# julius-speech/julius

Hardware: NVIDIA H100
Metric: frames/sec (xRT) 20k-word triphone decode (higher is better)
Workload: dtype f32

## Files before the change

### julius_b200/csrc/beam.cu

```cuda
#include "common.cuh"
#include "heap_pipe.cuh"
#include <vector>
#include <algorithm>

struct jb200_gmm;
struct jb200_dnn;
namespace jb200 {
int dnn_forward_device(jb200_dnn *h, const float *d_in, int T, float *d_rows, int row_stride, cudaStream_t st);
int gmm_device(const jb200_gmm *h);
int gmm_dim(const jb200_gmm *h);
int gmm_launch_states(jb200_gmm *h, const float *d_feats, int T, float *d_rows, int row_stride, cudaStream_t st,
                      const int *seg_off, const int *seg_start, int n_seg);
int gmm_cd_device(const jb200_gmm *h, const int **cd_off, const int **cd_states, int *method, int *nbest);

static constexpr int BEAM_THREADS = 256;
static constexpr int NWARP = BEAM_THREADS / 32;
static constexpr int SEQ_LOCAL_BITS = 18;
static constexpr unsigned SEQ_LOCAL = 1u << SEQ_LOCAL_BITS;
static constexpr int CD_NMAX = 16;
static constexpr int MAX_WORDS = 150;

struct __align__(16) NodeRec { float self_a, next_a; int arc_off, arc_n; int stend, next; int scid, out; };
struct __align__(8) Tok { float score; int node; int tre; int cword; float lscore; int tre_wid; };
struct __align__(16) Cand { float score; int node; float lscore; int src; };
// ... 162 lines not shown
        }
      }
      if (n < maxn) n++;
    }
  }
  float prob = 0.0f;
  for (int i = 0; i < n; i++) prob += mp[i];
  return prob / (float)n;
}

__device__ __forceinline__ float outprob_style(const BeamParams &p, const float *__restrict__ row, int out, int last_wid) {
  const int style = (unsigned)out >> 28, ref = out & 0x0fffffff;
  if (style == JB200_AS_STATE) return __ldg(row + ref);
  if (style == JB200_AS_LSET) return cdset_score(p, row, ref);
  const int col = (last_wid < 0) ? p.n_ctx : __ldg(p.word_ctx + last_wid);
  const int r = __ldg(p.rset_ctx + (size_t)ref * (p.n_ctx + 1) + col);
  if (r >= 0) return __ldg(row + r);
  return cdset_score(p, row, -r - 1);
}

__device__ __forceinline__ int block_excl_scan(int v, int *warp_sums, int *total) {
  const int lane = threadIdx.x & 31, wid = threadIdx.x >> 5;
  int x = v;
#pragma unroll
  for (int o = 1; o < 32; o <<= 1) { int y = __shfl_up_sync(0xffffffffu, x, o); if (lane >= o) x += y; }
  if (lane == 31) warp_sums[wid] = x;
  __syncthreads();
  if (wid == 0) {
    int s = (lane < NWARP) ? warp_sums[lane] : 0;
#pragma unroll
    for (int o = 1; o < 32; o <<= 1) { int y = __shfl_up_sync(0xffffffffu, s, o); if (lane >= o) s += y; }
    if (lane < NWARP) warp_sums[lane] = s;
  }
  __syncthreads();
  const int base = (wid == 0) ? 0 : warp_sums[wid - 1];
  *total = warp_sums[NWARP - 1];
  const int r = base + x - v;
  __syncthreads();
  return r;
}

__device__ __forceinline__ void cand_atomics(const SlotView &slots,
                                             int node, float score, unsigned seq_first, unsigned seq_win) {
  atomicMin(slots.fs(node), (int)seq_first);
  unsigned long long key = ((unsigned long long)fkey(score) << 32) | (unsigned)(~seq_win);
  atomicMax(slots.bk(node), key);
}

__device__ __forceinline__ float hval(unsigned long long e) { return __uint_as_float((unsigned)(e & 0xffffffffu)); }

template <bool MAXHEAP>
__device__ __forceinline__ bool hcmp(float a, float b) { return MAXHEAP ? (a < b) : (a > b); }
template <bool MAXHEAP>
__device__ __forceinline__ bool hstop(float s, float c) { return MAXHEAP ? (s >= c) : (s <= c); }

template <bool MAXHEAP>
__device__ __forceinline__ void sift_down(unsigned long long *A, int start, int n) {
  const unsigned long long s = A[start];
  const float sv = hval(s);
  int parent = start, child;
  while ((child = parent * 2) <= n) {
    const ulonglong2 pr = *reinterpret_cast<const ulonglong2 *>(A + child);
    unsigned long long c = pr.x;
    if (child < n && hcmp<MAXHEAP>(hval(pr.x), hval(pr.y))) { child++; c = pr.y; }
    if (hstop<MAXHEAP>(sv, hval(c))) break;
    A[parent] = c;
    parent = child;
  }
  A[parent] = s;
}

template <bool MAXHEAP>
__device__ __forceinline__ void sift_root_2level(unsigned long long *A, const unsigned long long s, const int m) {
  const float sv = hval(s);
  int parent = 1;
  while (true) {
    int child = parent * 2;
    if (child > m) break;
    const ulonglong2 pr = *reinterpret_cast<const ulonglong2 *>(A + child);
    const int g = parent * 4;
    ulonglong2 g01 = make_ulonglong2(0ull, 0ull), g23 = make_ulonglong2(0ull, 0ull);
    if (g <= m) g01 = *reinterpret_cast<const ulonglong2 *>(A + g);
    if (g + 2 <= m) g23 = *reinterpret_cast<const ulonglong2 *>(A + g + 2);
    unsigned long long c = pr.x; bool right = false;
    if (child < m && hcmp<MAXHEAP>(hval(pr.x), hval(pr.y))) { right = true; c = pr.y; }
    if (hstop<MAXHEAP>(sv, hval(c))) break;
    A[parent] = c;
    parent = child + (right ? 1 : 0);
    child = parent * 2;
    if (child > m) break;
    const ulonglong2 q = right ? g23 : g01;
    unsigned long long c2 = q.x; bool right2 = false;
    if (child < m && hcmp<MAXHEAP>(hval(q.x), hval(q.y))) { right2 = true; c2 = q.y; }
    if (hstop<MAXHEAP>(sv, hval(c2))) break;
    A[parent] = c2;
    parent = child + (right2 ? 1 : 0);
  }
  A[parent] = s;
}

template <bool MAXHEAP>
__device__ void heap_build(unsigned long long *A, int n) {
  const int half = n >> 1;
  if (half >= 1) {
    for (int L = 31 - __clz(half); L >= 0; L--) {
      const int lo = 1 << L;
      const int hi = min((2 << L) - 1, half);
      for (int i = lo + (int)threadIdx.x; i <= hi; i += BEAM_THREADS) sift_down<MAXHEAP>(A, i, n);
      __syncthreads();
    }
  }
}

template <bool MAXHEAP>
__device__ void heap_extract_seq(unsigned long long *A, int n, int extract) {
  if (threadIdx.x == 0) {
    int m = n;
    while (m > n - extract) {
      const unsigned long long s = A[m];
      A[m] = A[1];
      m--;
      if (m >= 1) sift_root_2level<MAXHEAP>(A, s, m);
    }
  }
  __syncthreads();
}

__device__ __forceinline__ ulonglong2 ldcg_pair(const unsigned long long *p) {
  const uint4 v = __ldcg(reinterpret_cast<const uint4 *>(p));
  return make_ulonglong2(((unsigned long long)v.y << 32) | v.x, ((unsigned long long)v.w << 32) | v.z);
}
struct HeapCache {
  unsigned long long *top; int cs;
  unsigned long long *tail; int tail_first, tail_n;
};

template <bool MAXHEAP>
__device__ void heap_extract_pipe_global(unsigned long long *A, const int n, const int extract, const float lose_below,
                                         unsigned long long *outs, const int maxt, const HeapCache hc,
                                         unsigned &ticks_out, unsigned &stalls_out) {
  constexpr int NL = 16;
  constexpr unsigned FULL = 0xffffffffu;
  const unsigned lane = threadIdx.x & 31;
  const unsigned long long sent = MAXHEAP ? 0xff800000ull : 0x7f800000ull;
  const int cap = (maxt >> 1) + 1;
  auto load_slot = [&](int i) -> unsigned long long {
    if (i < hc.cs) return hc.top[i];
    if (i >= hc.tail_first && i < hc.tail_first + hc.tail_n) return hc.tail[i - hc.tail_first];
    return __ldcg(A + i);
  };
  auto store_slot = [&](int i, unsigned long long v) {
    __stcg(A + i, v);
    if (i < hc.cs) hc.top[i] = v;
    else if (i >= hc.tail_first && i < hc.tail_first + hc.tail_n) hc.tail[i - hc.tail_first] = v;
  };
  bool act = false;
  int slot = 0, cur = cap, my_x = 0;
  unsigned long long s = sent;
  int next_x = 0, wait = 0;
  unsigned ticks = 0, stalls = 0;
  if (lane == 0 && extract > 0) outs[0] = load_slot(1);
  unsigned long long nxt = load_slot(n);
  while (true) {
    ulonglong2 pr = make_ulonglong2(sent, sent);
    if (act) {
      const int i = 2 * cur;
      if (i + 1 < hc.cs) pr = *reinterpret_cast<const ulonglong2 *>(hc.top + i);
      else if (i >= hc.tail_first && i + 1 < hc.tail_first + hc.tail_n) pr = make_ulonglong2(hc.tail[i - hc.tail_first], hc.tail[i + 1 - hc.tail_first]);
      else pr = ldcg_pair(A + i);
    }
    if (act) {
      const float xv = hval(pr.x), yv = hval(pr.y), sv = hval(s);
      const bool right = hcmp<MAXHEAP>(xv, yv);
      const unsigned long long c = right ? pr.y : pr.x;
      const float cv = hval(c);
      const bool stop = hstop<MAXHEAP>(sv, cv) || (MAXHEAP && cv < lose_below);
      const unsigned long long put = stop ? s : c;
      store_slot(slot, put);
      if (slot == 1) outs[my_x + 1] = put;
      if (stop) act = false;
      else { slot = 2 * cur + (right ? 1 : 0); cur = min(slot, cap); }
    }
    __syncwarp();
    if (--wait <= 0) {
      if (next_x >= extract) { if (!__any_sync(FULL, act)) break; }
      else {
        const int ms = n - next_x;
        const int ln = next_x & (NL - 1);
        bool blocks = act && ((int)lane == ln);
        if (!(MAXHEAP && hval(nxt) < lose_below)) {
          const int dh = 31 - __clz(max(slot, 1)), dms = 31 - __clz(ms);
          blocks = blocks || (act && dms >= dh && (ms >> (dms - dh)) == slot);
        }
        if (!__any_sync(FULL, blocks)) {
          if ((int)lane == ln) {
            s = load_slot(ms);
            store_slot(ms, sent);
            my_x = next_x; act = true; slot = 1; cur = 1;
          }
          next_x++; wait = 2;
          nxt = load_slot(n - next_x);
        } else stalls++;
      }
    }
    __syncwarp();
    ticks++;
  }
  ticks_out = ticks; stalls_out = stalls;
}

struct SlotClear {
  const Tok *tok; int n; SlotView slots;
  __device__ __forceinline__ void run(int first, int stride) const {
    for (int i = first; i < n; i += stride) {
      const int node = tok[i].node;
      slots.reset(node);
    }
  }
};

template <bool MAXHEAP>
__device__ __forceinline__ void heap_pad_sentinels(unsigned long long *A, const int n, const int maxt) {
  const unsigned long long sent = MAXHEAP ? 0xff800000ull : 0x7f800000ull;
  const int hi = min(2 * n + 1, maxt + 1);
  for (int i = n + 1 + (int)threadIdx.x; i <= hi; i += BEAM_THREADS) A[i] = sent;
  if (threadIdx.x < 2) A[maxt + 2 + threadIdx.x] = sent;
}

extern __shared__ __align__(16) unsigned char beam_smem[];
struct CutAreas {
  unsigned long long *heap;
  int *offs;
  unsigned long long *gq; int gqn;
  unsigned long long *gtail; int gtn;
  __device__ __forceinline__ unsigned long long *outv() const { return reinterpret_cast<unsigned long long *>(offs); }
};
__device__ __forceinline__ CutAreas cut_areas(const BeamParams &p) {
  unsigned long long *const smem_q = reinterpret_cast<unsigned long long *>(beam_smem);
  CutAreas a;
  a.heap = p.heap_g ? p.heap_g + (size_t)blockIdx.x * (p.maxt + 4) : smem_q;
  a.offs = reinterpret_cast<int *>(smem_q + (p.heap_g ? p.qcap : p.maxt + 4));
  a.gq = p.heap_g ? smem_q : nullptr;
  a.gqn = p.heap_g ? p.qcap : 0;
  a.gtail = p.heap_g ? reinterpret_cast<unsigned long long *>(a.offs + 2 * (p.beam + 2)) : nullptr;
  a.gtn = p.heap_g ? p.beam + 1 : 0;
  return a;
}

template <bool MAXHEAP>
__device__ void heap_extract_fast(const CutAreas &ca, const int n, const int extract, const float lose_below, const int maxt,
                                  unsigned long long *stats, const SlotClear *idle_work = nullptr) {
  unsigned long long *const A = ca.heap, *const outv = ca.outv(), *const gcache = ca.gq;
  HeapCache hc{nullptr, 0, nullptr, 0, 0};
  if (!__isShared(A) && n + 8 <= ca.gqn) {
    const int lmaxt = (ca.gqn - 4) & ~1;
    for (int i = threadIdx.x; i <= n; i += BEAM_THREADS) gcache[i] = A[i];
    heap_pad_sentinels<MAXHEAP>(gcache, n, lmaxt);
    __syncthreads();
    if (threadIdx.x >= 32 && idle_work) idle_work->run((int)threadIdx.x - 32, BEAM_THREADS - 32);
    if (threadIdx.x < 32) {
      unsigned ticks, stalls;
      heap_extract_pipe_warp6<MAXHEAP>(gcache, n, extract, lose_below, outv, lmaxt, threadIdx.x, ticks, stalls);
      if (threadIdx.x == 0) {
        atomicAdd(stats + CUT_REPLAY_TICKS, (unsigned long long)ticks); atomicAdd(stats + CUT_REPLAY_EXTRACTS, (unsigned long long)extract);
        atomicAdd(stats + CUT_HELD_BACK, (unsigned long long)stalls); atomicAdd(stats + CUT_GLOBAL_WHOLE, 1ull);
      }
    }
    __syncthreads();
    for (int i = 1 + threadIdx.x; i <= n; i += BEAM_THREADS) A[i] = gcache[i];
    __syncthreads();
    return;
  }
  if (!__isShared(A)) {
    hc.top = gcache; hc.cs = min(ca.gqn, maxt + 4) & ~1;
    for (int i = threadIdx.x; i < hc.cs; i += BEAM_THREADS) gcache[i] = A[i];
    if (ca.gtn >= extract) {
      hc.tail = ca.gtail; hc.tail_first = n - extract + 1; hc.tail_n = extract;
      for (int i = threadIdx.x; i < extract; i += BEAM_THREADS) ca.gtail[i] = A[hc.tail_first + i];
    }
    __syncthreads();
  }
  if (threadIdx.x >= 32 && idle_work) idle_work->run((int)threadIdx.x - 32, BEAM_THREADS - 32);
  if (threadIdx.x < 32) {
    unsigned ticks, stalls;
    if (!__isShared(A)) heap_extract_pipe_global<MAXHEAP>(A, n, extract, lose_below, outv, maxt, hc, ticks, stalls);
    else heap_extract_pipe_warp6<MAXHEAP>(A, n, extract, lose_below, outv, maxt, threadIdx.x, ticks, stalls);
    if (threadIdx.x == 0) {
      atomicAdd(stats + CUT_REPLAY_TICKS, (unsigned long long)ticks); atomicAdd(stats + CUT_REPLAY_EXTRACTS, (unsigned long long)extract);
      atomicAdd(stats + CUT_HELD_BACK, (unsigned long long)stalls);
      if (!__isShared(A)) atomicAdd(stats + CUT_GLOBAL_TOP_TAIL, 1ull);
    }
  }
  __syncthreads();
}

__device__ __forceinline__ int closed_subtree_size(const int c, const int n, const int H) {
  const int dc = 31 - __clz(c);
  if (dc > H) return 0;
  const int sh = H - dc;
  const int first = c << sh, width = 1 << sh;
  return (width - 1) + max(0, min(n - first + 1, width));
}

__device__ __noinline__ int closed_relocate(unsigned long long *keys, const int nc, const int n, const int need, unsigned *flags, unsigned *multi,
                                            unsigned *pay, const int lane) {
  constexpr unsigned FULL = 0xffffffffu;
  const int H = 31 - __clz(n);
  const int tail0 = n - need + 1, fwords = (need + 31) >> 5;
  for (int w = fwords - 1; w >= 0; w--) {
    unsigned bits = flags[w];
    while (bits) {
      const int b = 31 - __clz(bits);
      const int m = tail0 + w * 32 + b;
      const int k = n - m + 1;
      if (m <= n && m >= 2 && k <= need) {
        const int dm = 31 - __clz(m);
        const bool is_multi = (multi[(m - tail0) >> 5] >> ((m - tail0) & 31)) & 1u;
        int j = 0, a = 1, lo = 0, hi = n, occ = -1;
        bool gone = false;
        for (int base = k - 1; base < nc && occ < 0 && !gone; base += 32) {
          const int idx = base + lane;
          const unsigned long long key = (idx < nc) ? keys[idx] : 0ull;
          const int pre = 0xffff - (int)((key >> 16) & 0xffffu);
          unsigned done = 0u;
          while (true) {
            const bool in = (idx < nc) && pre >= lo && pre < hi && !((done >> lane) & 1u);
            const unsigned mask = __ballot_sync(FULL, in);
            if (!mask) break;
            const int f = __ffs(mask) - 1;
            if (j == dm) { occ = base + f; break; }
            if (!is_multi && (int)(pay[(unsigned)keys[base + f] & 0xffffu] >> 16) == m) { gone = true; break; }
            j++;
            const int nxt = m >> (dm - j);
            const int lsz = closed_subtree_size(2 * a, n, H);
            if (nxt == 2 * a) { lo = lo + 1; hi = lo + lsz; } else { lo = lo + 1 + lsz; }
            a = nxt;
            done |= (f >= 31) ? FULL : ((2u << f) - 1u);
          }
        }
        if (occ >= k) {
          __syncwarp();
          const unsigned long long ekey = keys[occ];
          const unsigned esc = (unsigned)(ekey >> 32);
          const int msz = m - 1;
          int x = 1; lo = 0; hi = n;
          bool stop = (2 * x > msz);
          for (int base = k; base < nc && !stop; base += 32) {
            const int idx = base + lane;
            const unsigned long long key = (idx < nc) ? keys[idx] : 0ull;
            const int pre = 0xffff - (int)((key >> 16) & 0xffffu);
            unsigned done = 0u;
            while (!stop) {
              const bool in = (idx < nc) && idx != occ && pre >= lo && pre < hi && !((done >> lane) & 1u);
              const unsigned mask = __ballot_sync(FULL, in);
              if (!mask) break;
              const int f = __ffs(mask) - 1;
              const unsigned osc = __shfl_sync(FULL, (unsigned)(key >> 32), f);
              const int opre = __shfl_sync(FULL, pre, f);
              if (opre == lo) return 0;
              if (esc >= osc) { stop = true; break; }
              const int lsz = closed_subtree_size(2 * x, n, H);
              if (opre < lo + 1 + lsz) { x = 2 * x; lo = lo + 1; hi = lo + lsz; }
              else { x = 2 * x + 1; lo = lo + 1 + lsz; }
              if (2 * x > msz) { stop = true; break; }
              done |= (f >= 31) ? FULL : ((2u << f) - 1u);
            }
          }
          const unsigned long long nkey = (ekey & 0xffffffff0000ffffull) | ((unsigned long long)(0xffffu - (unsigned)lo) << 16);
          int cnt = 0;
          {
            const int wb = max(k, occ - 16), we = wb + 31;
            const bool lo_ok = (wb == k) || ((unsigned)(keys[wb] >> 32) > esc);
            const bool hi_ok = (we >= nc) || ((unsigned)(keys[we] >> 32) < esc);
            if (lo_ok && hi_ok) {
              const int idx = wb + lane;
              const bool gt = (idx < nc) && idx != occ && keys[idx] > nkey;
              cnt = (wb - k) + __popc(__ballot_sync(FULL, gt));
            } else {
              for (int base = k; base < nc; base += 32) {
                const int idx = base + lane;
                const bool gt = (idx < nc) && idx != occ && keys[idx] > nkey;
                const unsigned mask = __ballot_sync(FULL, gt);
                cnt += __popc(mask);
                const bool le = (idx < nc) && idx != occ && !gt;
                if (__any_sync(FULL, le)) break;
              }
            }
          }
          const int ins = k + cnt;
          if (ins < occ) {
            for (int top = occ; top > ins; top -= 32) {
              const int idx = top - lane;
              unsigned long long v = 0ull;
              if (idx > ins) v = keys[idx - 1];
              __syncwarp();
              if (idx > ins) keys[idx] = v;
              __syncwarp();
            }
          } else if (ins > occ) {
            for (int bot = occ; bot < ins; bot += 32) {
              const int idx = bot + lane;
              unsigned long long v = 0ull;
              if (idx < ins) v = keys[idx + 1];
              __syncwarp();
              if (idx < ins) keys[idx] = v;
              __syncwarp();
            }
          }
          if (lane == 0) {
            keys[ins] = nkey;
            unsigned *pp = pay + ((unsigned)nkey & 0xffffu);
            *pp = ((unsigned)x << 16) | (*pp & 0xffffu);
            if (x >= tail0 && x < m) { flags[(x - tail0) >> 5] |= 1u << ((x - tail0) & 31); multi[(x - tail0) >> 5] |= 1u << ((x - tail0) & 31); }
          }
          __syncwarp();
        }
      }
      bits = flags[w] & ((b == 0) ? 0u : ((1u << b) - 1u));
    }
  }
  return 1;
}

__device__ int heap_select_closed(unsigned long long *heap, const int n, const int need, const float lose_below, const int maxt,
                                  unsigned long long *keys, const int key_cap, unsigned *pay, const int pay_cap,
                                  int *ordn, int *s_scratch ) {
  const int tid = threadIdx.x;
  int relocated = 0;
  if (n >= 65536 || maxt >= 65536 || !(lose_below > -INFINITY)) return 0;
  const int tail0 = n - need + 1, fwords = (need + 31) >> 5;
  unsigned *const flags = pay + pay_cap - fwords, *const multi = pay + pay_cap - 2 * fwords;
  const bool have_flags = (2 * fwords < pay_cap);
  if (tid == 0) { s_scratch[0] = 0; s_scratch[1] = 0; }
  if (have_flags) for (int i = tid; i < 2 * fwords; i += BEAM_THREADS) multi[i] = 0u;
  __syncthreads();
  const int H = 31 - __clz(n);
  const int cap = min(min(key_cap, have_flags ? pay_cap - 2 * fwords : pay_cap), 65535);
  for (int h0 = 1; h0 <= n; h0 += BEAM_THREADS) {
    const int h = h0 + tid;
    unsigned long long e = 0ull;
    bool is_c = false;
    if (h <= n) { e = heap[h]; is_c = (hval(e) >= lose_below); }
    const unsigned m = __ballot_sync(0xffffffffu, is_c);
    int base = 0;
    if ((tid & 31) == 0 && m) base = atomicAdd(&s_scratch[0], __popc(m));
    base = __shfl_sync(0xffffffffu, base, 0);
    if (is_c) {
      const int ci = base + __popc(m & ((1u << (tid & 31)) - 1u));
      if (ci < cap) {
        int pre = 0, cur = 1;
        for (int b = (31 - __clz(h)) - 1; b >= 0; b--) {
          const int bit = (h >> b) & 1;
          pre += 1 + (bit ? closed_subtree_size(cur * 2, n, H) : 0);
          cur = cur * 2 + bit;
        }
        keys[ci] = ((unsigned long long)fkey(hval(e)) << 32) | ((unsigned long long)(0xffffu - (unsigned)pre) << 16) | (unsigned)ci;
        pay[ci] = ((unsigned)h << 16) | (unsigned)(e >> 32);
      }
    }
  }
  __syncthreads();
  const int nc = s_scratch[0];
  int np = 1; while (np < nc) np <<= 1;
  if (nc > cap || np > key_cap || nc < need) return 0;
  const bool can_relocate = have_flags;
  for (int i = nc + tid; i < np; i += BEAM_THREADS) keys[i] = 0ull;
  __syncthreads();
  for (int k = 2; k <= np; k <<= 1) {
    for (int j = k >> 1; j > 0; j >>= 1) {
      for (int i = tid; i < (np >> 1); i += BEAM_THREADS) {
        const int a = ((i & ~(j - 1)) << 1) | (i & (j - 1)), b = a | j;
        const unsigned long long ka = keys[a], kb = keys[b];
        const bool desc = ((a & k) == 0);
        if (desc ? (ka < kb) : (ka > kb)) { keys[a] = kb; keys[b] = ka; }
      }
      __syncthreads();
    }
  }
  const unsigned theta = (unsigned)(keys[need - 1] >> 32);
  for (int i = tid; i < nc; i += BEAM_THREADS) {
    const unsigned long long ki = keys[i];
    const unsigned sk = (unsigned)(ki >> 32);
    if (sk < theta) continue;
    const int slot = (int)(pay[(unsigned)ki & 0xffffu] >> 16);
    if (slot < tail0) continue;
    const bool tied = (i > 0 && (unsigned)(keys[i - 1] >> 32) == sk) || (i + 1 < nc && (unsigned)(keys[i + 1] >> 32) == sk);
    int last = i;
    if (tied) { int g = 0; while (last + 1 < nc && (unsigned)(keys[last + 1] >> 32) == sk && g < 8) { last++; g++; } if (g == 8) last = nc; }
    const int kstep = n - slot + 1, d = 31 - __clz(slot);
    if (last + 1 < kstep + d) continue;
    if (have_flags) atomicOr(flags + ((slot - tail0) >> 5), 1u << ((slot - tail0) & 31));
    if (tied) s_scratch[1] = 1;
  }
  __syncthreads();
  if (s_scratch[1]) {
    if (!can_relocate) return 0;
    if (tid < 32) { const int ok = closed_relocate(keys, nc, n, need, flags, multi, pay, tid); if (tid == 0) s_scratch[1] = ok ? 2 : 1; }
    __syncthreads();
    if (s_scratch[1] != 2) return 0;
    relocated = 1;
  }
  for (int k = tid; k < need; k += BEAM_THREADS) ordn[k] = (int)(pay[(unsigned)keys[need - 1 - k] & 0xffffu] & 0xffffu);
  return 1 + relocated;
}


__device__ int trace_backptr(const jb200_atom *atoms, int a, int *w) {
  int n = 0;
  w[n++] = atoms[a].wid;
  while (atoms[a].begintime > 0) {
    a = atoms[a].last;
    if (a < 0 || n >= MAX_WORDS) break;
    w[n++] = atoms[a].wid;
  }
  for (int i = 0; i < n / 2; i++) { const int x = w[i]; w[i] = w[n - 1 - i]; w[n - 1 - i] = x; }
  return n;
}

__device__ void interim_best(const BeamParams &p, const int u, const jb200_atom *araw, const int lo, const int hi, const int frame) {
  UttState *st = p.state + u;
  int best = -1; float mx = JB200_LOG_ZERO;
  for (int a = hi - 1; a >= lo; a--) if (mx < araw[a].backscore) { mx = araw[a].backscore; best = a; }
  st->interim_frame = frame - 1;
  if (best < 0) { st->interim_nwords = 0; st->interim_score = JB200_LOG_ZERO; return; }
  st->interim_nwords = trace_backptr(araw, best, p.interim_words + (size_t)u * MAX_WORDS); st->interim_score = mx;
}

#define PROF_MARK(k) do { if (tid == 0) { long long _n = clock64(); s_prof[k] += _n - s_tprev; s_tprev = _n; } } while (0)

__device__ __forceinline__ void beam_cut(const BeamParams &p, const CutAreas &ca, const int n, const unsigned &s_maxkey,
                                         const Tok *tn, const SlotView &slots, int *ordn, long long *s_prof, long long &s_tprev) {
  __shared__ unsigned s_losekey;
  __shared__ int s_cf[2];
  const int tid = threadIdx.x;
  const int need = p.beam, maxt = p.maxt;
  unsigned long long *const heap = ca.heap, *const outv = ca.outv();
  const SlotClear sc{tn, n, slots};
  if (need < n - need) {
    constexpr int NB = 1024;
    int *hist = ca.offs;
    const int nb = min(NB, 2 * (p.beam + 2));
    for (int i = tid; i < nb; i += BEAM_THREADS) hist[i] = 0;
    __syncthreads();
    const unsigned maxkey = s_maxkey;
    const int e = (int)((((maxkey & 0x80000000u) ? (maxkey & 0x7fffffffu) : ~maxkey) >> 23) & 0xffu) - 127;
    const int sh = max(0, min(24, 22 - e));
    for (int r = tid; r < n; r += BEAM_THREADS) {
      const unsigned key = fkey(hval(heap[r + 1]));
      const unsigned bin = min((unsigned)(nb - 1), (maxkey - key) >> sh);
      atomicAdd(&hist[bin], 1);
    }
    __syncthreads();
    if (tid < 32) {
      int cum = 0, found = -1;
      for (int b0 = 0; b0 < nb && found < 0; b0 += 32) {
        const int v = (b0 + tid < nb) ? hist[b0 + tid] : 0;
        int x = v;
        for (int o = 1; o < 32; o <<= 1) { int y = __shfl_up_sync(0xffffffffu, x, o); if (tid >= o) x += y; }
        const unsigned hit = __ballot_sync(0xffffffffu, cum + x >= need);
        if (hit) found = b0 + __ffs(hit) - 1;
        cum += __shfl_sync(0xffffffffu, x, 31);
      }
      if (tid == 0) {
        unsigned lk = 0u;
        if (found >= 0 && found < nb - 1) {
          const unsigned long long drop = (unsigned long long)(found + 1) << sh;
          lk = (drop < maxkey) ? maxkey - (unsigned)drop : 0u;
        }
        s_losekey = lk;
      }
    }
    __syncthreads();
    const unsigned lk = s_losekey;
    const float lose_below = (lk == 0u) ? -INFINITY : __uint_as_float((lk & 0x80000000u) ? (lk & 0x7fffffffu) : ~lk);
    heap_build<true>(heap, n); PROF_MARK(7);
    sc.run(tid, BEAM_THREADS);
    const int closed = heap_select_closed(heap, n, need, lose_below, maxt, ca.gq ? ca.gq : heap + n + 1, ca.gq ? p.sort_cap : maxt + 3 - n,
                                          reinterpret_cast<unsigned *>(ca.offs), 2 * (p.beam + 2), ordn, s_cf);
    if (tid == 0) {
      atomicAdd(p.cut_counters + CUT_UPWARD, 1ull);
      if (closed) atomicAdd(p.cut_counters + CUT_CLOSED, 1ull);
      if (closed == 2) atomicAdd(p.cut_counters + CUT_RELOCATED, 1ull);
    }
    if (!closed) {
      heap_pad_sentinels<true>(heap, n, maxt);
      __syncthreads();
      heap_extract_fast<true>(ca, n, need, lose_below, maxt, p.cut_counters);
      for (int k = tid; k < need; k += BEAM_THREADS) ordn[k] = (int)(outv[need - 1 - k] >> 32);
    }
  } else {
    heap_pad_sentinels<false>(heap, n, maxt);
    heap_build<false>(heap, n); PROF_MARK(7);
    heap_extract_fast<false>(ca, n, n - need, -INFINITY, maxt, p.cut_counters, &sc);
    for (int k = tid; k < need; k += BEAM_THREADS) ordn[k] = (int)(heap[k + 1] >> 32);
  }
}

template <bool GRAMMAR>
__device__ __forceinline__ void finalize_utt(const BeamParams &p, const int u, const int tid, const int T, jb200_atom *araw, int *newidx,
                                             const int *group0, jb200_utt_result *res, int *words,
                                             int &s_natoms, int &s_overflow, int &s_found, long long &s_outbase,
                                             long long *s_prof, long long &s_tprev) {
  const int natoms = s_natoms;
  for (int a = tid; a < natoms; a += BEAM_THREADS) {
    const jb200_atom me = araw[a];
    const int lo = group0[me.endtime], hi = group0[me.endtime + 1];
    int rank = 0;
    for (int b = lo; b < hi; b++) rank += (araw[b].wid < me.wid) ? 1 : 0;
    newidx[a] = lo + rank;
  }
  if (tid == 0) {
    if (p.atoms_in_place) s_outbase = p.atom_off[u];
    else {
      unsigned long long base = atomicAdd(p.atom_counter, (unsigned long long)natoms);
      if ((long long)(base + natoms) > p.atoms_out_cap) { s_overflow = 1; s_outbase = -1; }
      else s_outbase = (long long)base;
    }
  }
  __syncthreads();
  const long long ob = s_outbase;
  const bool can_write = (ob >= 0);
  const int kept = can_write ? natoms : 0;
  for (int a = tid; a < kept; a += BEAM_THREADS) {
    jb200_atom me = araw[a];
    me.last = (me.last < 0) ? -1 : newidx[me.last];
    p.atoms_out[ob + newidx[a]] = me;
    if ((GRAMMAR || me.wid == p.tail_silwid) && me.backscore > JB200_LOG_ZERO) atomicMax(&s_found, me.endtime);
  }
  __threadfence_block();
  __syncthreads();

  if (tid == 0) {
    int status = 0, nw = 0; float score = 0.0f;
    const int last_time = s_found;
    if (kept == 0 || last_time < 0) status = -1;
    else {
      const jb200_atom *const atoms = p.atoms_out + ob;
      const int lo = group0[last_time], hi = group0[last_time + 1];
      int best = -1;
      if constexpr (GRAMMAR) {
        float maxscore = JB200_LOG_ZERO;
        for (int b = lo; b < hi; b++) {
          const jb200_atom x = atoms[b];
          if (maxscore < x.backscore) { maxscore = x.backscore; best = b; }
        }
      } else {
        for (int b = lo; b < hi; b++) {
          const jb200_atom x = atoms[b];
          if (x.wid == p.tail_silwid && x.backscore > JB200_LOG_ZERO) { best = b; break; }
        }
      }
      if (best < 0) status = -1;
      else { nw = trace_backptr(atoms, best, words); score = atoms[best].backscore; }
    }
    jb200_utt_result r;
    r.status = status; r.n_frames = T; r.n_atoms = kept; r.n_words = nw; r.score = score;
    r.atom_offset = ob; r.word_offset = u * MAX_WORDS; r.overflow = s_overflow;
    *res = r;
    PROF_MARK(7);
    if (p.prof) for (int k = 0; k < 8; k++) p.prof[(size_t)u * 8 + k] = s_prof[k];
  }
}

struct UttAreas {
  Tok *tok0; int *ord0; SlotView slots; Cand *cand; CandB *candb; IsoCand *iso; WEnd *wend;
  Tok *surv;
  unsigned *bits; int *wpre;
  jb200_atom *araw; int *newidx; int atom_cap;
  int *group0;
  int *counts; jb200_utt_result *res; int *words;
};
__device__ __forceinline__ UttAreas utt_areas(const BeamParams &p, const int u) {
  const int f_begin = p.frame_off[u];
  const long long a0 = p.atom_off[u];
  UttAreas a;
  a.tok0 = p.tok + (size_t)u * 2 * p.maxt;
  a.ord0 = p.order + (size_t)u * 2 * p.maxt;
  a.slots = SlotView{p.slots + (size_t)u * p.n_nodes};
  a.cand = p.cand + (size_t)u * p.maxc;
  a.candb = p.candb + (size_t)u * p.maxc;
  a.surv = p.surv + (size_t)u * (p.beam + 2);
  a.iso = p.iso + (size_t)u * max(max(p.n_iso, p.n_isoarc), 1);
  a.wend = p.wend + (size_t)u * p.maxw;
  a.bits = p.bitmask + (size_t)u * (p.maxbits >> 5);
  a.wpre = p.wordpre + (size_t)u * (p.maxbits >> 5);
  a.atom_cap = (int)(p.atom_off[u + 1] - a0);
  a.araw = p.atoms_raw + a0;
  a.newidx = p.newidx + a0;
  a.group0 = p.group0 + (size_t)f_begin + u;
  a.counts = p.counts + (size_t)f_begin * 2;
  a.res = p.results + u;
  a.words = p.words + (size_t)u * MAX_WORDS;
  return a;
}

__device__ __forceinline__ void resume_scalars(const bool first, const UttState *ust, int &natoms, int &overflow, float &thr, int &ns,
                                               long long *prof) {
  if (first) { natoms = 0; overflow = 0; thr = JB200_LOG_ZERO; ns = 0; for (int k = 0; k < 8; k++) prof[k] = 0; }
  else { natoms = ust->natoms; overflow = ust->overflow; thr = ust->thr; ns = ust->ns; for (int k = 0; k < 8; k++) prof[k] = ust->prof[k]; }
}

__device__ __forceinline__ void park_scalars(const BeamParams &p, const int u, const UttAreas &ua, const int T, const int natoms,
                                             const int overflow, const float thr, const int ns, const int cur, const int tnum_prev,
                                             const int stopped, const bool slots_clean, long long *prof, const long long tprev) {
  UttState *const ust = p.state + u;
  ust->natoms = natoms; ust->overflow = overflow; ust->thr = thr; ust->ns = ns; ust->cur = cur;
  ust->tnum_prev = tnum_prev; ust->stopped = stopped; ust->slots_clean = slots_clean ? 1 : 0;
  ust->t_done = T;
  long long _n = clock64(); prof[7] += _n - tprev;
  for (int k = 0; k < 8; k++) ust->prof[k] = prof[k];
  if (p.interim) interim_best(p, u, ua.araw, (T >= 2 && stopped < 0) ? ua.group0[T - 2] : natoms, natoms, T - 1);
}

__device__ __forceinline__ jb200_atom trellis_atom(const Tok &tk, const int wid, const int endtime, const jb200_atom *araw) {
  jb200_atom a;
  a.wid = wid; a.backscore = tk.score;
  a.begintime = (tk.tre < 0 ? -1 : araw[tk.tre].endtime) + 1;
  a.endtime = endtime; a.last = tk.tre; a.lscore = tk.lscore;
  return a;
}

struct IntraArc { int next; float score, lscore; int out; };
__device__ __forceinline__ IntraArc intra_arc(const BeamParams &p, const Tok &tk, const NodeRec &nr, const int k) {
  int next; float pa;
  const int has_self = (nr.self_a != JB200_LOG_ZERO), has_next = (nr.next_a != JB200_LOG_ZERO);
  if (has_self && k == 0) { next = tk.node; pa = nr.self_a; }
  else if (has_next && k == has_self) { next = nr.next; pa = nr.next_a; }
  else { const int a = k - has_self - has_next; next = __ldg(p.arc_to + nr.arc_off + a); pa = __ldg(p.arc_a + nr.arc_off + a); }
  float tmpsum = tk.score + pa;
  float lsc = JB200_LOG_ZERO;
  int out_next = nr.out;
  if (next != tk.node) {
    const int2 so = __ldg(reinterpret_cast<const int2 *>(&p.nodes[next].scid));
    const int scid = so.x;
    out_next = so.y;
    if (scid != 0) {
      lsc = max_successor_prob(p, tk.cword, scid) * p.lm_weight + p.lm_penalty;
      tmpsum -= tk.lscore;
      tmpsum += lsc;
    }
  }
  if (lsc == JB200_LOG_ZERO) lsc = tk.lscore;
  return IntraArc{next, tmpsum, lsc, out_next};
}

__device__ __forceinline__ int rank_creators(const unsigned *bits, int *wpre, const int nwords, int *s_warp) {
  int carry = 0;
  for (int w0 = 0; w0 < nwords; w0 += BEAM_THREADS) {
    const int w = w0 + (int)threadIdx.x;
    const int cnt = (w < nwords) ? __popc(__ldcg(bits + w)) : 0;
    int tot;
    const int ex = block_excl_scan(cnt, s_warp, &tot);
    if (w < nwords) wpre[w] = carry + ex;
    carry += tot;
  }
  return carry;
}

__device__ __forceinline__ void end_frame(const BeamParams &p, int *counts, const int t, const int ncre, const int ns_new,
                                          const unsigned pmaxkey, int &ns, float &thr) {
  counts[2 * t] = ncre; counts[2 * t + 1] = ns_new;
  ns = ns_new;
  if (p.prune_width >= 0.0f && pmaxkey != 0u) {
    const unsigned b = (pmaxkey & 0x80000000u) ? (pmaxkey & 0x7fffffffu) : ~pmaxkey;
    thr = __uint_as_float(b) - p.prune_width;
  } else thr = JB200_LOG_ZERO;
}

__device__ __noinline__ void check_select(unsigned long long *chk, const int n, const int need, const Tok *tok,
                                          const unsigned long long *heap, const int *ordn, int *overflow) {
  if (!overflow) {
    for (int h = 1 + (int)threadIdx.x; h <= n; h += BEAM_THREADS) chk[h] = heap[h];
    __syncthreads();
    return;
  }
  const bool upward = (need < n - need);
  __syncthreads();
  if (tok) for (int r = threadIdx.x; r < n; r += BEAM_THREADS) chk[r + 1] = ((unsigned long long)(unsigned)r << 32) | __float_as_uint(tok[r].score);
  __syncthreads();
  if (upward) { heap_build<true>(chk, n); heap_extract_seq<true>(chk, n, need); }
  else { heap_build<false>(chk, n); heap_extract_seq<false>(chk, n, n - need); }
  bool bad = false;
  if (heap) {
    for (int h = 1 + (int)threadIdx.x; h <= n; h += BEAM_THREADS) bad |= (chk[h] != heap[h]);
  } else {
    const int start = upward ? n - need : 0;
    for (int k = threadIdx.x; k < need; k += BEAM_THREADS) bad |= (ordn[k] != (int)(chk[start + k + 1] >> 32));
  }
  if (bad) *overflow = 4;
  __syncthreads();
}

static constexpr int BEAM_MINBLOCKS = 4;
template <bool GRAMMAR, bool CHECK>
__global__ void __launch_bounds__(BEAM_THREADS, BEAM_MINBLOCKS)
beam_kernel(const BeamParams p) {
  const int u = blockIdx.x;
  const int tid = threadIdx.x;
  const ChunkDesc ck = p.chunk[u];
  if (ck.flags & CHUNK_SKIP) return;
// ... 1545 lines not shown
```

Baseline: 1.115 million.

## Parallelize closed-heap relocation across warps and sort small stages in registers

Closed-heap relocation was done by a single warp. It is now split into an occupant search, run in parallel by up to eight warps on candidate slots, and a serial reinsert done by warp 0, with block-level sync between rounds. The bitonic sort now handles stages up to 128 elements inside each warp using registers and shuffles, so those stages skip shared-memory passes and per-stage __syncthreads. The cost is more block barriers in the relocation loop, plus speculative occupant searches that are wasted when an earlier slot gets reinserted first.

```diff
diff --git a/julius_b200/csrc/beam.cu b/julius_b200/csrc/beam.cu
--- a/julius_b200/csrc/beam.cu
+++ b/julius_b200/csrc/beam.cu
@@ -488,124 +488,197 @@
   return (width - 1) + max(0, min(n - first + 1, width));
 }
 
+__device__ int relocate_occupant(const unsigned long long *keys, const int nc, const int n, const int H, const int m, const int k,
+                                 const bool is_multi, const unsigned *pay, const int lane) {
+  constexpr unsigned FULL = 0xffffffffu;
+  const int dm = 31 - __clz(m);
+  int j = 0, a = 1, lo = 0, hi = n, occ = -1;
+  bool gone = false;
+  for (int base = k - 1; base < nc && occ < 0 && !gone; base += 32) {
+    const int idx = base + lane;
+    const unsigned long long key = (idx < nc) ? keys[idx] : 0ull;
+    const int pre = 0xffff - (int)((key >> 16) & 0xffffu);
+    unsigned done = 0u;
+    while (true) {
+      const bool in = (idx < nc) && pre >= lo && pre < hi && !((done >> lane) & 1u);
+      const unsigned mask = __ballot_sync(FULL, in);
+      if (!mask) break;
+      const int f = __ffs(mask) - 1;
+      if (j == dm) { occ = base + f; break; }
+      if (!is_multi && (int)(pay[(unsigned)keys[base + f] & 0xffffu] >> 16) == m) { gone = true; break; }
+      j++;
+      const int nxt = m >> (dm - j);
+      const int lsz = closed_subtree_size(2 * a, n, H);
+      if (nxt == 2 * a) { lo = lo + 1; hi = lo + lsz; } else { lo = lo + 1 + lsz; }
+      a = nxt;
+      done |= (f >= 31) ? FULL : ((2u << f) - 1u);
+    }
+  }
+  return gone ? -1 : occ;
+}
+
+__device__ int relocate_reinsert(unsigned long long *keys, const int nc, const int n, const int H, const int need, const int m,
+                                 const int k, const int occ, unsigned *flags, unsigned *multi, unsigned *pay, const int lane) {
+  constexpr unsigned FULL = 0xffffffffu;
+  const int tail0 = n - need + 1;
+  __syncwarp();
+  const unsigned long long ekey = keys[occ];
+  const unsigned esc = (unsigned)(ekey >> 32);
+  const int msz = m - 1;
+  int x = 1, lo = 0, hi = n;
+  bool stop = (2 * x > msz);
+  for (int base = k; base < nc && !stop; base += 32) {
+    const int idx = base + lane;
+    const unsigned long long key = (idx < nc) ? keys[idx] : 0ull;
+    const int pre = 0xffff - (int)((key >> 16) & 0xffffu);
+    unsigned done = 0u;
+    while (!stop) {
+      const bool in = (idx < nc) && idx != occ && pre >= lo && pre < hi && !((done >> lane) & 1u);
+      const unsigned mask = __ballot_sync(FULL, in);
+      if (!mask) break;
+      const int f = __ffs(mask) - 1;
+      const unsigned osc = __shfl_sync(FULL, (unsigned)(key >> 32), f);
+      const int opre = __shfl_sync(FULL, pre, f);
+      if (opre == lo) return 0;
+      if (esc >= osc) { stop = true; break; }
+      const int lsz = closed_subtree_size(2 * x, n, H);
+      if (opre < lo + 1 + lsz) { x = 2 * x; lo = lo + 1; hi = lo + lsz; }
+      else { x = 2 * x + 1; lo = lo + 1 + lsz; }
+      if (2 * x > msz) { stop = true; break; }
+      done |= (f >= 31) ? FULL : ((2u << f) - 1u);
+    }
+  }
+  const unsigned long long nkey = (ekey & 0xffffffff0000ffffull) | ((unsigned long long)(0xffffu - (unsigned)lo) << 16);
+  int cnt = 0;
+  {
+    const int wb = max(k, occ - 16), we = wb + 31;
+    const bool lo_ok = (wb == k) || ((unsigned)(keys[wb] >> 32) > esc);
+    const bool hi_ok = (we >= nc) || ((unsigned)(keys[we] >> 32) < esc);
+    if (lo_ok && hi_ok) {
+      const int idx = wb + lane;
+      const bool gt = (idx < nc) && idx != occ && keys[idx] > nkey;
+      cnt = (wb - k) + __popc(__ballot_sync(FULL, gt));
+    } else {
+      for (int base = k; base < nc; base += 32) {
+        const int idx = base + lane;
+        const bool gt = (idx < nc) && idx != occ && keys[idx] > nkey;
+        const unsigned mask = __ballot_sync(FULL, gt);
+        cnt += __popc(mask);
+        const bool le = (idx < nc) && idx != occ && !gt;
+        if (__any_sync(FULL, le)) break;
+      }
+    }
+  }
+  const int ins = k + cnt;
+  if (ins < occ) {
+    for (int top = occ; top > ins; top -= 32) {
+      const int idx = top - lane;
+      unsigned long long v = 0ull;
+      if (idx > ins) v = keys[idx - 1];
+      __syncwarp();
+      if (idx > ins) keys[idx] = v;
+      __syncwarp();
+    }
+  } else if (ins > occ) {
+    for (int bot = occ; bot < ins; bot += 32) {
+      const int idx = bot + lane;
+      unsigned long long v = 0ull;
+      if (idx < ins) v = keys[idx + 1];
+      __syncwarp();
+      if (idx < ins) keys[idx] = v;
+      __syncwarp();
+    }
+  }
+  if (lane == 0) {
+    keys[ins] = nkey;
+    unsigned *pp = pay + ((unsigned)nkey & 0xffffu);
+    *pp = ((unsigned)x << 16) | (*pp & 0xffffu);
+    if (x >= tail0 && x < m) { flags[(x - tail0) >> 5] |= 1u << ((x - tail0) & 31); multi[(x - tail0) >> 5] |= 1u << ((x - tail0) & 31); }
+  }
+  __syncwarp();
+  return 1;
+}
+
+constexpr int RELOC_WARPS = BEAM_THREADS / 32;
 __device__ __noinline__ int closed_relocate(unsigned long long *keys, const int nc, const int n, const int need, unsigned *flags, unsigned *multi,
-                                            unsigned *pay, const int lane) {
-  constexpr unsigned FULL = 0xffffffffu;
+                                            unsigned *pay) {
+  __shared__ int s_m[RELOC_WARPS], s_occ[RELOC_WARPS], s_ok;
+  const int tid = threadIdx.x, warp = tid >> 5, lane = tid & 31;
   const int H = 31 - __clz(n);
-  const int tail0 = n - need + 1, fwords = (need + 31) >> 5;
-  for (int w = fwords - 1; w >= 0; w--) {
-    unsigned bits = flags[w];
-    while (bits) {
-      const int b = 31 - __clz(bits);
-      const int m = tail0 + w * 32 + b;
-      const int k = n - m + 1;
-      if (m <= n && m >= 2 && k <= need) {
-        const int dm = 31 - __clz(m);
-        const bool is_multi = (multi[(m - tail0) >> 5] >> ((m - tail0) & 31)) & 1u;
-        int j = 0, a = 1, lo = 0, hi = n, occ = -1;
-        bool gone = false;
-        for (int base = k - 1; base < nc && occ < 0 && !gone; base += 32) {
-          const int idx = base + lane;
-          const unsigned long long key = (idx < nc) ? keys[idx] : 0ull;
-          const int pre = 0xffff - (int)((key >> 16) & 0xffffu);
-          unsigned done = 0u;
-          while (true) {
-            const bool in = (idx < nc) && pre >= lo && pre < hi && !((done >> lane) & 1u);
-            const unsigned mask = __ballot_sync(FULL, in);
-            if (!mask) break;
-            const int f = __ffs(mask) - 1;
-            if (j == dm) { occ = base + f; break; }
-            if (!is_multi && (int)(pay[(unsigned)keys[base + f] & 0xffffu] >> 16) == m) { gone = true; break; }
-            j++;
-            const int nxt = m >> (dm - j);
-            const int lsz = closed_subtree_size(2 * a, n, H);
-            if (nxt == 2 * a) { lo = lo + 1; hi = lo + lsz; } else { lo = lo + 1 + lsz; }
-            a = nxt;
-            done |= (f >= 31) ? FULL : ((2u << f) - 1u);
+  const int tail0 = n - need + 1;
+  int below = need;
+  while (true) {
+    if (tid == 0) {
+      int c = 0;
+      for (int r = below - 1; r >= 0 && c < RELOC_WARPS; ) {
+        const unsigned bits = flags[r >> 5] & ((2u << (r & 31)) - 1u);
+        if (!bits) { r = (r & ~31) - 1; continue; }
+        const int b = 31 - __clz(bits);
+        r = (r & ~31) + b;
+        const int m = tail0 + r;
+        if (m <= n && m >= 2 && n - m + 1 <= need) s_m[c++] = m;
+        r--;
+      }
+      for (; c < RELOC_WARPS; c++) s_m[c] = 0;
+    }
+    __syncthreads();
+    const int m = s_m[warp];
+    if (m) {
+      const bool is_multi = (multi[(m - tail0) >> 5] >> ((m - tail0) & 31)) & 1u;
+      const int occ = relocate_occupant(keys, nc, n, H, m, n - m + 1, is_multi, pay, lane);
+      if (lane == 0) s_occ[warp] = occ;
+    }
+    __syncthreads();
+    int w = 0;
+    while (w < RELOC_WARPS && s_m[w] && s_occ[w] < n - s_m[w] + 1) w++;
+    if (w == RELOC_WARPS || !s_m[w]) {
+      if (w < RELOC_WARPS || !s_m[RELOC_WARPS - 1]) return 1;
+      below = s_m[RELOC_WARPS - 1] - tail0;
+      __syncthreads();
+      continue;
+    }
+    const int me = s_m[w];
+    if (warp == 0) {
+      const int ok = relocate_reinsert(keys, nc, n, H, need, me, n - me + 1, s_occ[w], flags, multi, pay, lane);
+      if (lane == 0) s_ok = ok;
+    }
+    __syncthreads();
+    if (!s_ok) return 0;
+    below = me - tail0;
+  }
+}
+
+constexpr int SORT_TILE = 128;
+__device__ __forceinline__ void sort_cx(unsigned long long &a, unsigned long long &b, const bool desc) {
+  const unsigned long long hi = a > b ? a : b, lo = a > b ? b : a;
+  a = desc ? hi : lo; b = desc ? lo : hi;
+}
+__device__ __noinline__ void sort_tiles(unsigned long long *keys, const int np, const int k0, const int k1) {
+  const int lane = threadIdx.x & 31;
+  const int np_t = max(np, SORT_TILE);
+  for (int base = (threadIdx.x >> 5) * SORT_TILE; base < np_t; base += BEAM_THREADS / 32 * SORT_TILE) {
+    unsigned long long x[4];
+#pragma unroll
+    for (int q = 0; q < 4; q++) { const int e = base + 32 * q + lane; x[q] = (e < np) ? keys[e] : 0ull; }
+    for (int k = k0; k <= k1; k <<= 1) {
+      for (int j = min(k >> 1, 64); j > 0; j >>= 1) {
+        if (j == 64) {
+          sort_cx(x[0], x[2], ((base + lane) & k) == 0); sort_cx(x[1], x[3], ((base + 32 + lane) & k) == 0);
+        } else if (j == 32) {
+          sort_cx(x[0], x[1], ((base + lane) & k) == 0); sort_cx(x[2], x[3], ((base + 64 + lane) & k) == 0);
+        } else {
+#pragma unroll
+          for (int q = 0; q < 4; q++) {
+            const unsigned long long o = __shfl_xor_sync(0xffffffffu, x[q], j);
+            const bool keep_hi = ((((base + 32 * q + lane) & k) == 0) == ((lane & j) == 0));
+            x[q] = (keep_hi == (x[q] > o)) ? x[q] : o;
           }
         }
-        if (occ >= k) {
-          __syncwarp();
-          const unsigned long long ekey = keys[occ];
-          const unsigned esc = (unsigned)(ekey >> 32);
-          const int msz = m - 1;
-          int x = 1; lo = 0; hi = n;
-          bool stop = (2 * x > msz);
-          for (int base = k; base < nc && !stop; base += 32) {
-            const int idx = base + lane;
-            const unsigned long long key = (idx < nc) ? keys[idx] : 0ull;
-            const int pre = 0xffff - (int)((key >> 16) & 0xffffu);
-            unsigned done = 0u;
-            while (!stop) {
-              const bool in = (idx < nc) && idx != occ && pre >= lo && pre < hi && !((done >> lane) & 1u);
-              const unsigned mask = __ballot_sync(FULL, in);
-              if (!mask) break;
-              const int f = __ffs(mask) - 1;
-              const unsigned osc = __shfl_sync(FULL, (unsigned)(key >> 32), f);
-              const int opre = __shfl_sync(FULL, pre, f);
-              if (opre == lo) return 0;
-              if (esc >= osc) { stop = true; break; }
-              const int lsz = closed_subtree_size(2 * x, n, H);
-              if (opre < lo + 1 + lsz) { x = 2 * x; lo = lo + 1; hi = lo + lsz; }
-              else { x = 2 * x + 1; lo = lo + 1 + lsz; }
-              if (2 * x > msz) { stop = true; break; }
-              done |= (f >= 31) ? FULL : ((2u << f) - 1u);
-            }
-          }
-          const unsigned long long nkey = (ekey & 0xffffffff0000ffffull) | ((unsigned long long)(0xffffu - (unsigned)lo) << 16);
-          int cnt = 0;
-          {
-            const int wb = max(k, occ - 16), we = wb + 31;
-            const bool lo_ok = (wb == k) || ((unsigned)(keys[wb] >> 32) > esc);
-            const bool hi_ok = (we >= nc) || ((unsigned)(keys[we] >> 32) < esc);
-            if (lo_ok && hi_ok) {
-              const int idx = wb + lane;
-              const bool gt = (idx < nc) && idx != occ && keys[idx] > nkey;
-              cnt = (wb - k) + __popc(__ballot_sync(FULL, gt));
-            } else {
-              for (int base = k; base < nc; base += 32) {
-                const int idx = base + lane;
-                const bool gt = (idx < nc) && idx != occ && keys[idx] > nkey;
-                const unsigned mask = __ballot_sync(FULL, gt);
-                cnt += __popc(mask);
-                const bool le = (idx < nc) && idx != occ && !gt;
-                if (__any_sync(FULL, le)) break;
-              }
-            }
-          }
-          const int ins = k + cnt;
-          if (ins < occ) {
-            for (int top = occ; top > ins; top -= 32) {
-              const int idx = top - lane;
-              unsigned long long v = 0ull;
-              if (idx > ins) v = keys[idx - 1];
-              __syncwarp();
-              if (idx > ins) keys[idx] = v;
-              __syncwarp();
-            }
-          } else if (ins > occ) {
-            for (int bot = occ; bot < ins; bot += 32) {
-              const int idx = bot + lane;
-              unsigned long long v = 0ull;
-              if (idx < ins) v = keys[idx + 1];
-              __syncwarp();
-              if (idx < ins) keys[idx] = v;
-              __syncwarp();
-            }
-          }
-          if (lane == 0) {
-            keys[ins] = nkey;
-            unsigned *pp = pay + ((unsigned)nkey & 0xffffu);
-            *pp = ((unsigned)x << 16) | (*pp & 0xffffu);
-            if (x >= tail0 && x < m) { flags[(x - tail0) >> 5] |= 1u << ((x - tail0) & 31); multi[(x - tail0) >> 5] |= 1u << ((x - tail0) & 31); }
-          }
-          __syncwarp();
-        }
-      }
-      bits = flags[w] & ((b == 0) ? 0u : ((1u << b) - 1u));
-    }
-  }
-  return 1;
+      }
+    }
+#pragma unroll
+    for (int q = 0; q < 4; q++) { const int e = base + 32 * q + lane; if (e < np) keys[e] = x[q]; }
+  }
 }
 
 __device__ int heap_select_closed(unsigned long long *heap, const int n, const int need, const float lose_below, const int maxt,
@@ -652,8 +725,8 @@
   const bool can_relocate = have_flags;
   for (int i = nc + tid; i < np; i += BEAM_THREADS) keys[i] = 0ull;
   __syncthreads();
-  for (int k = 2; k <= np; k <<= 1) {
-    for (int j = k >> 1; j > 0; j >>= 1) {
+  for (int k = SORT_TILE; k <= max(np, SORT_TILE); k <<= 1) {
+    for (int j = k >> 1; j >= SORT_TILE; j >>= 1) {
       for (int i = tid; i < (np >> 1); i += BEAM_THREADS) {
         const int a = ((i & ~(j - 1)) << 1) | (i & (j - 1)), b = a | j;
         const unsigned long long ka = keys[a], kb = keys[b];
@@ -662,6 +735,8 @@
       }
       __syncthreads();
     }
+    sort_tiles(keys, np, k == SORT_TILE ? 2 : k, k);
+    __syncthreads();
   }
   const unsigned theta = (unsigned)(keys[need - 1] >> 32);
   for (int i = tid; i < nc; i += BEAM_THREADS) {
@@ -681,7 +756,8 @@
   __syncthreads();
   if (s_scratch[1]) {
     if (!can_relocate) return 0;
-    if (tid < 32) { const int ok = closed_relocate(keys, nc, n, need, flags, multi, pay, tid); if (tid == 0) s_scratch[1] = ok ? 2 : 1; }
+    const int ok = closed_relocate(keys, nc, n, need, flags, multi, pay);
+    if (tid == 0) s_scratch[1] = ok ? 2 : 1;
     __syncthreads();
     if (s_scratch[1] != 2) return 0;
     relocated = 1;
```

Measured after the change: 1.188 million (median of 6 runs). 6.6% higher.
